# Lucaskabela/UNAST

Hardware: AMD Instinct MI355X
Metric: mel-frames/sec/node (train step, gen+disc) at B=32,T_mel=800; 1/2/4/8-GPU scaling (higher is better)
Workload: dtype bf16x3

## Files before the change

### unast_amd/csrc/panel.hip

```cpp
#include "common.h"
#include <algorithm>
#include "../../include/unast_hip.h"
#include <type_traits>

static unsigned long long* g_panel_stamps = nullptr;
#define PSUB 1024

struct PanelParams {
    const float* A; int lda;
    const unsigned char* W; size_t plane_bytes;
    float* C; int ldc;
    int M, N, K, ncg;
    const float* bias; const float* R; int ldr;
    const float* G; int ldg; float gate_scale;
    int act; uint32_t drop_thresh; float drop_scale; uint32_t seed, stream;
    int out_split;
    const float* gamma; const float* beta; float* Y; int ldy; float* mean; float* rstd; float eps;
    const float* Z; int ldz; float* part;
    unsigned long long* gate_bits;
    unsigned long long* stamps;
};

__device__ __forceinline__ void panel_wait_vm(int n) {
#define PW(k) asm volatile("s_waitcnt vmcnt(" #k ")" ::: "memory")
// ... 356 lines not shown
                        x += rr[r];
                        zv[rt][cg][c2][r] = x;
                        s1[rt] += x;
                    }
                }
            s1[rt] += __shfl_xor(s1[rt], 16, 64);
            s1[rt] += __shfl_xor(s1[rt], 32, 64);
        }
        if (g == 0) {
#pragma unroll
            for (int rt = 0; rt < RT; ++rt) sred[((rg * 2 + ch) * RT + rt) * 16 + l15] = s1[rt];
        }
        __syncthreads();
        float mu[RT], s2[RT];
#pragma unroll
        for (int rt = 0; rt < RT; ++rt) {
            mu[rt] = (s1[rt] + sred[((rg * 2 + (ch ^ 1)) * RT + rt) * 16 + l15]) * (1.f / 256.f);
            s2[rt] = 0.f;
#pragma unroll
            for (int cg = 0; cg < 4; ++cg)
#pragma unroll
                for (int c2 = 0; c2 < 2; ++c2)
#pragma unroll
                    for (int r = 0; r < 4; ++r) { const float d = zv[rt][cg][c2][r] - mu[rt]; s2[rt] += d * d; }
            s2[rt] += __shfl_xor(s2[rt], 16, 64);
            s2[rt] += __shfl_xor(s2[rt], 32, 64);
        }
        __syncthreads();
        if (g == 0) {
#pragma unroll
            for (int rt = 0; rt < RT; ++rt) sred[((rg * 2 + ch) * RT + rt) * 16 + l15] = s2[rt];
        }
        __syncthreads();
#pragma unroll
        for (int rt = 0; rt < RT; ++rt) {
            const int m = m_wave + 16 * rt + l15;
            const float rs = rsqrtf((s2[rt] + sred[((rg * 2 + (ch ^ 1)) * RT + rt) * 16 + l15]) * (1.f / 256.f) + p.eps);
            if (m >= p.M) continue;
            if (g == 0 && ch == 0) { p.mean[m] = mu[rt]; p.rstd[m] = rs; }
#pragma unroll
            for (int cg = 0; cg < 4; ++cg)
#pragma unroll
                for (int c2 = 0; c2 < 2; ++c2) {
                    const int n = 64 * cg + 32 * ch + 16 * c2 + 4 * g;
                    const float4 g4 = *reinterpret_cast<const float4*>(p.gamma + n), b4 = *reinterpret_cast<const float4*>(p.beta + n);
                    const float* z = zv[rt][cg][c2];
                    *reinterpret_cast<float4*>(p.C + (size_t)m * p.ldc + n) = make_float4(z[0], z[1], z[2], z[3]);
                    *reinterpret_cast<float4*>(p.Y + (size_t)m * p.ldy + n) =
                        make_float4((z[0] - mu[rt]) * rs * g4.x + b4.x, (z[1] - mu[rt]) * rs * g4.y + b4.y, (z[2] - mu[rt]) * rs * g4.z + b4.z, (z[3] - mu[rt]) * rs * g4.w + b4.w);
                }
        }
    } else {
        const bool late = ((wave >> 2) & 1) != 0;
        f32x4 acc[RT][2], pend[RT][2];
        zero(acc);
        for (int cg = 0; cg < p.ncg; ++cg) {
            group_sync(cg);
            if (!late && cg > 0) run_epilogue(cg - 1, pend);
            group_mma(cg, I0{}, IH{}, acc);
            if (late && cg > 0) run_epilogue(cg - 1, pend);
            group_mma(cg, IH{}, IK{}, acc);
            end_iteration();
#pragma unroll
            for (int rt = 0; rt < RT; ++rt) { pend[rt][0] = acc[rt][0]; pend[rt][1] = acc[rt][1]; }
            zero(acc);
        }
        run_epilogue(p.ncg - 1, pend);
    }
    asm volatile("s_waitcnt vmcnt(0)" ::: "memory");
#ifdef PANEL_STAMPS
    if (p.stamps && lane == 0) {
        stamp_sum[6] = panel_stamp() - t_begin;
        for (int k = 0; k < 8; ++k) p.stamps[((size_t)blockIdx.x * 8 + wave) * 8 + k] = stamp_sum[k];
    }
#endif
}

typedef __attribute__((ext_vector_type(16))) float f32x16_t;
__global__ __launch_bounds__(512, 1) void panel32_kernel(const PanelParams p) {
    constexpr int KSTEPS = 8, NW = 8, NT = 64 * NW, ROWS = 128;
    constexpr int NSUB = 8 * KSTEPS, GROUP = NSUB * PSUB, DMAX = NSUB / NW, RING = 2 * GROUP;
    static_assert(RING >= ROWS * 1024, "the A image borrows the ring");
    __shared__ __attribute__((aligned(16))) unsigned char smem[RING + 4096 + 1024];
    const int t = threadIdx.x, lane = t & 63, l31 = lane & 31, kh = lane >> 5;
    const int wave = __builtin_amdgcn_readfirstlane(t >> 6);
    __builtin_assume(wave >= 0 && wave < NW);
    const int rg = wave >> 1, ch = wave & 1;
    const int m_wg = blockIdx.x * ROWS, m_wave = m_wg + 32 * rg;
    const uint32_t rbase = p.drop_thresh ? rng_stream_base(p.seed, p.stream) : 0u;
    const __amdgpu_buffer_rsrc_t w_rsrc = __builtin_amdgcn_make_buffer_rsrc(const_cast<unsigned char*>(p.W), 0, 0x7FFFFFF0, 0x00020000);
    const int lane16 = lane * 16;
    auto issue_group = [&](int cg) {
#pragma unroll
        for (int q = 0; q < DMAX; ++q) {
            const int j = wave + NW * q;
            const int pl = j / (4 * KSTEPS), rem = j - pl * (4 * KSTEPS);
            const uint32_t soff = (uint32_t)pl * (uint32_t)p.plane_bytes + (uint32_t)(4 * cg * KSTEPS + rem) * PSUB;
            __builtin_amdgcn_raw_ptr_buffer_load_lds(w_rsrc, (__attribute__((address_space(3))) void*)(smem + (cg & 1) * GROUP + j * PSUB), 16, lane16, (int)soff, 0, 0);
        }
    };
    float* const sbias = reinterpret_cast<float*>(smem + RING);
    const uint32_t sbias_lds = (uint32_t)(uintptr_t)(__attribute__((address_space(3))) void*)sbias;
    const bool bias_lds = p.bias != nullptr;
    if (bias_lds) for (int i = t; i < 64 * p.ncg; i += NT) sbias[i] = (i < p.N) ? p.bias[i] : 0.f;

    bf16x8_t ah[16], al[16];
    {
        const __amdgpu_buffer_rsrc_t a_rsrc = __builtin_amdgcn_make_buffer_rsrc(const_cast<float*>(p.A), 0, 0x7FFFFFF0, 0x00020000);
#pragma unroll
        for (int q = 0; q < ROWS / NW; ++q) {
            const int r = wave * (ROWS / NW) + q;
            const int row = min(m_wg + r, p.M - 1);
            __builtin_amdgcn_raw_ptr_buffer_load_lds(a_rsrc, (__attribute__((address_space(3))) void*)(smem + r * 1024), 16, (lane ^ (r & 15)) << 4,
                                                     (int)((uint32_t)row * (uint32_t)p.lda * 4u), 0, 0);
        }
        asm volatile("s_waitcnt vmcnt(0)" ::: "memory");
        __syncthreads();
        const unsigned char* rowp = smem + (32 * rg + l31) * 1024;
        const int sw = l31 & 15;
#pragma unroll
        for (int ks = 0; ks < 16; ++ks) {
            const int c0 = 4 * ks + 2 * kh;
            const float4 a = *reinterpret_cast<const float4*>(rowp + ((c0 ^ sw) << 4));
            const float4 c = *reinterpret_cast<const float4*>(rowp + (((c0 + 1) ^ sw) << 4));
            u32x2 h0, l0, h1, l1;
            split4<3>(a, h0, l0);
            split4<3>(c, h1, l1);
            ah[ks] = __builtin_bit_cast(bf16x8_t, (u32x4){h0[0], h0[1], h1[0], h1[1]});
            al[ks] = __builtin_bit_cast(bf16x8_t, (u32x4){l0[0], l0[1], l1[0], l1[1]});
        }
        __syncthreads();
    }
    issue_group(0);

    const __amdgpu_buffer_rsrc_t c_rsrc = __builtin_amdgcn_make_buffer_rsrc(p.C, 0, (int)min((size_t)0x7FFFFFF0, ((size_t)(p.M - 1) * p.ldc + p.N) * 4), 0x00020000);
    const int m = m_wave + l31;
    const uint32_t c_voff = ((uint32_t)m * (uint32_t)p.ldc + (uint32_t)(32 * ch + 4 * kh)) * 4u;
    const uint32_t c_rkey = pcg_hash((uint32_t)m + rbase);
    auto epilogue = [&](int cg, const f32x16_t& ac, auto act_t, auto drop_t, auto split_t) {
        constexpr bool ACT = decltype(act_t)::value, DROP = decltype(drop_t)::value, SPLIT = decltype(split_t)::value;
        f32x4 b4[4];
#pragma unroll
        for (int j = 0; j < 4; ++j) b4[j] = (f32x4){0.f, 0.f, 0.f, 0.f};
        if (bias_lds) {
            const uint32_t ba = sbias_lds + 4u * (uint32_t)(64 * cg + 32 * ch + 4 * kh);
            asm volatile("ds_read_b128 %0, %4\n\tds_read_b128 %1, %4 offset:32\n\tds_read_b128 %2, %4 offset:64\n\tds_read_b128 %3, %4 offset:96\n\ts_waitcnt lgkmcnt(0)"
                         : "=&v"(b4[0]), "=&v"(b4[1]), "=&v"(b4[2]), "=&v"(b4[3]) : "v"(ba) : "memory");
        }
        const int soff = cg * 256;
#pragma unroll
        for (int j = 0; j < 4; ++j) {
            float v[4] = {ac[4 * j] + b4[j][0], ac[4 * j + 1] + b4[j][1], ac[4 * j + 2] + b4[j][2], ac[4 * j + 3] + b4[j][3]};
            if (ACT) {
#pragma unroll
                for (int r = 0; r < 4; ++r) asm("v_max_f32 %0, 0, %1" : "=v"(v[r]) : "v"(v[r]));
            }
            if (DROP) {
                const uint32_t n = (uint32_t)(64 * cg + 32 * ch + 8 * j + 4 * kh);
                const uint32_t h01 = rng_pair(c_rkey, n), h23 = rng_pair(c_rkey, n + 2u);
                v[0] = rng_keep_lo(h01, p.drop_thresh) ? v[0] * p.drop_scale : 0.f;
                v[1] = rng_keep_hi(h01, p.drop_thresh) ? v[1] * p.drop_scale : 0.f;
                v[2] = rng_keep_lo(h23, p.drop_thresh) ? v[2] * p.drop_scale : 0.f;
                v[3] = rng_keep_hi(h23, p.drop_thresh) ? v[3] * p.drop_scale : 0.f;
            }
            u32x4 o;
            if (SPLIT) {
                const uint4 sc = split_chunk(make_float4(v[0], v[1], v[2], v[3]));
                o = (u32x4){sc.x, sc.y, sc.z, sc.w};
            } else {
                o = (u32x4){__float_as_uint(v[0]), __float_as_uint(v[1]), __float_as_uint(v[2]), __float_as_uint(v[3])};
            }
            __builtin_amdgcn_raw_buffer_store_b128(o, c_rsrc, (int)(c_voff + (uint32_t)soff) + 32 * j, 0, 0);
        }
    };
    const int epi_kind = p.drop_thresh ? 1 : p.out_split ? 2 : p.act == 1 ? 3 : 4;
    int st_prev = 0, st_now = 0;
    auto run_epilogue = [&](int cg, const f32x16_t& ac) {
        using T = std::true_type; using F = std::false_type;
        __builtin_amdgcn_s_setprio(1);
        if (epi_kind == 1) epilogue(cg, ac, T{}, T{}, F{});
        else if (epi_kind == 2) epilogue(cg, ac, F{}, F{}, T{});
        else if (epi_kind == 3) epilogue(cg, ac, T{}, F{}, F{});
        else epilogue(cg, ac, F{}, F{}, F{});
        __builtin_amdgcn_s_setprio(0);
        st_now += 4;
    };
    auto group_sync = [&](int cg) {
        panel_wait_vm(st_prev);
        __builtin_amdgcn_s_barrier();
        if (cg + 1 < p.ncg) issue_group(cg + 1);
    };
    const int lane_off = (2 * ch + (l31 >> 4)) * KSTEPS * PSUB + (kh * 16 + (l31 & 15)) * 16;
    auto group_mma = [&](int cg, auto k0_t, auto k1_t, f32x16_t& ac) {
        constexpr int K0 = decltype(k0_t)::value, K1 = decltype(k1_t)::value;
        const unsigned char* base = smem + (cg & 1) * GROUP + lane_off;
        bf16x8_t bf[2][2];
        auto load_b = [&](int buf, int ks) {
            bf[buf][0] = *reinterpret_cast<const bf16x8_t*>(base + (ks >> 1) * PSUB + (ks & 1) * 512);
            bf[buf][1] = *reinterpret_cast<const bf16x8_t*>(base + 4 * KSTEPS * PSUB + (ks >> 1) * PSUB + (ks & 1) * 512);
        };
        load_b(K0 & 1, K0);
#pragma unroll
        for (int ks = K0; ks < K1; ++ks) {
            if (ks + 1 < K1) load_b((ks + 1) & 1, ks + 1);
            const bf16x8_t bh = bf[ks & 1][0], bl = bf[ks & 1][1];
            ac = __builtin_amdgcn_mfma_f32_32x32x16_bf16(bl, ah[ks], ac, 0, 0, 0);
            ac = __builtin_amdgcn_mfma_f32_32x32x16_bf16(bh, al[ks], ac, 0, 0, 0);
            ac = __builtin_amdgcn_mfma_f32_32x32x16_bf16(bh, ah[ks], ac, 0, 0, 0);
        }
    };
    using I0 = std::integral_constant<int, 0>; using IH = std::integral_constant<int, 8>; using IK = std::integral_constant<int, 16>;
    const bool late = ((wave >> 2) & 1) != 0;
    f32x16_t acc, pend;
#pragma unroll
    for (int i = 0; i < 16; ++i) { acc[i] = 0.f; pend[i] = 0.f; }
    for (int cg = 0; cg < p.ncg; ++cg) {
        group_sync(cg);
        if (!late && cg > 0) run_epilogue(cg - 1, pend);
        group_mma(cg, I0{}, IH{}, acc);
        if (late && cg > 0) run_epilogue(cg - 1, pend);
        group_mma(cg, IH{}, IK{}, acc);
        st_prev = st_now; st_now = 0;
        pend = acc;
#pragma unroll
        for (int i = 0; i < 16; ++i) acc[i] = 0.f;
    }
    run_epilogue(p.ncg - 1, pend);
    asm volatile("s_waitcnt vmcnt(0)" ::: "memory");
}

struct RetileDesc { int src_off, ld, transposed, N, K, n0, k0, ksteps; long long dst_off, plane_bytes; };

__global__ __launch_bounds__(256) void retile_kernel(const float* __restrict__ src_base, unsigned char* __restrict__ dst_base, const RetileDesc* __restrict__ descs) {
    __shared__ float tile[64][65];
    const RetileDesc d = descs[blockIdx.x];
    const float* src = src_base + d.src_off;
    const int t = threadIdx.x;
#pragma unroll
    for (int i = 0; i < 4; ++i) {
        const int idx = t + 256 * i, r = idx >> 4, c4 = (idx & 15) * 4;
        float v[4] = {0.f, 0.f, 0.f, 0.f};
        if (!d.transposed) {
            const int n = d.n0 + r;
            for (int e = 0; e < 4; ++e) if (n < d.N && d.k0 + c4 + e < d.K) v[e] = src[(size_t)n * d.ld + d.k0 + c4 + e];
            for (int e = 0; e < 4; ++e) tile[r][c4 + e] = v[e];
        } else {
            const int k = d.k0 + r;
            for (int e = 0; e < 4; ++e) if (k < d.K && d.n0 + c4 + e < d.N) v[e] = src[(size_t)k * d.ld + d.n0 + c4 + e];
            for (int e = 0; e < 4; ++e) tile[c4 + e][r] = v[e];
        }
    }
    __syncthreads();
#pragma unroll
    for (int i = 0; i < 2; ++i) {
        const int u = t + 256 * i;
        const int st = u >> 6, w = u & 63;
        const int ct = st >> 1, ksl = st & 1, gg = w >> 4, l = w & 15;
        const int ks = d.k0 / 32 + ksl;
        if (ks >= d.ksteps) continue;
        const int n = 16 * ct + l, k = 32 * ksl + 8 * gg;
        const float4 a = make_float4(tile[n][k], tile[n][k + 1], tile[n][k + 2], tile[n][k + 3]);
        const float4 c = make_float4(tile[n][k + 4], tile[n][k + 5], tile[n][k + 6], tile[n][k + 7]);
        u32x2 h0, l0, h1, l1;
        split4<3>(a, h0, l0);
        split4<3>(c, h1, l1);
        unsigned char* dst = dst_base + d.dst_off + ((size_t)((d.n0 / 16 + ct) * d.ksteps + ks)) * PSUB + w * 16;
        *reinterpret_cast<uint4*>(dst) = make_uint4(h0[0], h0[1], h1[0], h1[1]);
        *reinterpret_cast<uint4*>(dst + d.plane_bytes) = make_uint4(l0[0], l0[1], l1[0], l1[1]);
    }
}

extern "C" int unast_retile_weights(const float* src_base, void* dst_base, const void* descs_dev, int ndesc, hipStream_t stream) {
    UNAST_REQUIRE(src_base && dst_base && descs_dev && ndesc > 0, "unast_retile_weights: bad arguments");
    UNAST_REQUIRE((((uintptr_t)dst_base) & 15) == 0, "unast_retile_weights: destination must be 16-byte aligned");
    hipLaunchKernelGGL(retile_kernel, dim3(ndesc), dim3(256), 0, stream, src_base, (unsigned char*)dst_base, (const RetileDesc*)descs_dev);
    return unast_check_launch("unast_retile_weights");
}

template <int LN>
__global__ __launch_bounds__(1024, 4) void kpanel_kernel(const PanelParams p) {
    constexpr int NW = 16, ROWS = 128, WSLOT = 32768, ASLOT = 16384;
    __shared__ __attribute__((aligned(16))) unsigned char smem[3 * WSLOT + 3 * ASLOT + 1024 + 2048];
    const int t = threadIdx.x, lane = t & 63, l15 = lane & 15, g = lane >> 4;
    const int wave = __builtin_amdgcn_readfirstlane(t >> 6);
    __builtin_assume(wave >= 0 && wave < NW);
    const int rg = wave >> 2, ch = wave & 3;
    const int m_wg = blockIdx.x * ROWS, n_wg = blockIdx.y * 256;
    const int m_wave = m_wg + 32 * rg;
    const int KG = p.K >> 5;
#ifdef PANEL_STAMPS
    unsigned long long stamp_sum[8] = {0, 0, 0, 0, 0, 0, 0, 0};
    const unsigned long long t_begin = panel_stamp();
#endif
    const uint32_t rbase = p.drop_thresh ? rng_stream_base(p.seed, p.stream) : 0u;
    unsigned char* const aring = smem + 3 * WSLOT;

    const __amdgpu_buffer_rsrc_t w_rsrc = __builtin_amdgcn_make_buffer_rsrc(const_cast<unsigned char*>(p.W), 0, 0x7FFFFFF0, 0x00020000);
    const __amdgpu_buffer_rsrc_t a_rsrc = __builtin_amdgcn_make_buffer_rsrc(const_cast<float*>(p.A), 0, 0x7FFFFFF0, 0x00020000);
    const int lane16 = lane * 16;
    const int ar = 8 * wave + (lane >> 3);
    const uint32_t a_voff = ((uint32_t)min(m_wg + ar, p.M - 1) * (uint32_t)p.lda + 4u * (uint32_t)((lane & 7) ^ ((ar & 7) ^ ((ar >> 3) & 1)))) * 4u;
    const uint32_t w_soff0 = (uint32_t)((n_wg >> 4) + wave) * (uint32_t)(KG * PSUB);
    auto issue_group = [&](int kg, int slot) {
#pragma unroll
        for (int q = 0; q < 2; ++q)
            __builtin_amdgcn_raw_ptr_buffer_load_lds(w_rsrc, (__attribute__((address_space(3))) void*)(smem + slot * WSLOT + (q * 16 + wave) * PSUB), 16, lane16,
                                                     (int)((uint32_t)q * (uint32_t)p.plane_bytes + w_soff0 + (uint32_t)kg * PSUB), 0, 0);
        __builtin_amdgcn_raw_ptr_buffer_load_lds(a_rsrc, (__attribute__((address_space(3))) void*)(aring + slot * ASLOT + wave * 1024), 16, (int)a_voff, kg * 128, 0, 0);
    };
    float* const sbias = reinterpret_cast<float*>(smem + 3 * WSLOT + 3 * ASLOT);
    float* const sred = sbias + 256;
    if (t < 256) sbias[t] = p.bias ? p.bias[n_wg + t] : 0.f;
    issue_group(0, 0);
    if (KG > 1) issue_group(1, 1);

    f32x4 acc[2][4];
#pragma unroll
    for (int rt = 0; rt < 2; ++rt)
#pragma unroll
        for (int ct = 0; ct < 4; ++ct) acc[rt][ct] = (f32x4){0.f, 0.f, 0.f, 0.f};
    uint32_t a_rd[2][2];
#pragma unroll
    for (int rt = 0; rt < 2; ++rt) {
        const int r = 32 * rg + 16 * rt + l15, key = (r & 7) ^ ((r >> 3) & 1);
#pragma unroll
        for (int h = 0; h < 2; ++h) a_rd[rt][h] = (uint32_t)(r * 128 + (((2 * g + h) ^ key) << 4));
    }
    const uint32_t aring_lds = (uint32_t)(uintptr_t)(__attribute__((address_space(3))) void*)aring;
    const uint32_t wring_lds = (uint32_t)(uintptr_t)(__attribute__((address_space(3))) void*)smem + (uint32_t)(lane16 + (4 * ch) * PSUB);
    f32x4 raw[2][2];
    bf16x8_t b0h[2], b0l[2], b1h[2], b1l[2];
    bf16x8_t ah[2], al[2];
#define KP_READ_A(slot_) do { const uint32_t ab = aring_lds + (uint32_t)(slot_) * ASLOT; \
        asm volatile("ds_read_b128 %0, %4\n\tds_read_b128 %1, %5\n\tds_read_b128 %2, %6\n\tds_read_b128 %3, %7" \
                     : "=&v"(raw[0][0]), "=&v"(raw[0][1]), "=&v"(raw[1][0]), "=&v"(raw[1][1]) \
                     : "v"(ab + a_rd[0][0]), "v"(ab + a_rd[0][1]), "v"(ab + a_rd[1][0]), "v"(ab + a_rd[1][1]) : "memory"); } while (0)
#define KP_READ_W0(slot_) do { const uint32_t wb = wring_lds + (uint32_t)(slot_) * WSLOT; \
        asm volatile("ds_read_b128 %0, %4\n\tds_read_b128 %1, %4 offset:16384\n\tds_read_b128 %2, %4 offset:1024\n\tds_read_b128 %3, %4 offset:17408" \
                     : "=&v"(b0h[0]), "=&v"(b0l[0]), "=&v"(b0h[1]), "=&v"(b0l[1]) : "v"(wb) : "memory"); } while (0)
#define KP_READ_W1(slot_) do { const uint32_t wb = wring_lds + (uint32_t)(slot_) * WSLOT; \
        asm volatile("ds_read_b128 %0, %4 offset:2048\n\tds_read_b128 %1, %4 offset:18432\n\tds_read_b128 %2, %4 offset:3072\n\tds_read_b128 %3, %4 offset:19456" \
                     : "=&v"(b1h[0]), "=&v"(b1l[0]), "=&v"(b1h[1]), "=&v"(b1l[1]) : "v"(wb) : "memory"); } while (0)
    int slot = 0;
    if (KG > 1) asm volatile("s_waitcnt vmcnt(3)" ::: "memory"); else asm volatile("s_waitcnt vmcnt(0)" ::: "memory");
    __builtin_amdgcn_s_barrier();
    KP_READ_A(0);
    KP_READ_W0(0);
    if (KG > 2) issue_group(2, 2);
    for (int kg = 0; kg < KG; ++kg) {
        STAMP(ta);
        asm volatile("s_waitcnt lgkmcnt(4)" : "+v"(raw[0][0]), "+v"(raw[0][1]), "+v"(raw[1][0]), "+v"(raw[1][1]) :: "memory");
        STAMP(tb);
#pragma unroll
        for (int rt = 0; rt < 2; ++rt) {
            u32x2 h0, l0, h1, l1;
            split4<3>(make_float4(raw[rt][0][0], raw[rt][0][1], raw[rt][0][2], raw[rt][0][3]), h0, l0);
            split4<3>(make_float4(raw[rt][1][0], raw[rt][1][1], raw[rt][1][2], raw[rt][1][3]), h1, l1);
            ah[rt] = __builtin_bit_cast(bf16x8_t, (u32x4){h0[0], h0[1], h1[0], h1[1]});
            al[rt] = __builtin_bit_cast(bf16x8_t, (u32x4){l0[0], l0[1], l1[0], l1[1]});
        }
        KP_READ_W1(slot);
        asm volatile("s_waitcnt lgkmcnt(4)" : "+v"(b0h[0]), "+v"(b0l[0]), "+v"(b0h[1]), "+v"(b0l[1]) :: "memory");
        STAMP(tc);
#pragma unroll
        for (int ct = 0; ct < 2; ++ct)
#pragma unroll
            for (int rt = 0; rt < 2; ++rt) {
                acc[rt][ct] = mfma16(b0l[ct], ah[rt], acc[rt][ct]);
                acc[rt][ct] = mfma16(b0h[ct], al[rt], acc[rt][ct]);
                acc[rt][ct] = mfma16(b0h[ct], ah[rt], acc[rt][ct]);
            }
        asm volatile("" :: "v"(acc[0][0]), "v"(acc[1][0]), "v"(acc[0][1]), "v"(acc[1][1]));
        asm volatile("s_waitcnt lgkmcnt(0)" : "+v"(b1h[0]), "+v"(b1l[0]), "+v"(b1h[1]), "+v"(b1l[1]) :: "memory");
        STAMP(td);
        if (kg + 1 < KG) {
            if (kg + 2 < KG) asm volatile("s_waitcnt vmcnt(3)" ::: "memory"); else asm volatile("s_waitcnt vmcnt(0)" ::: "memory");
            STAMP(te);
            __builtin_amdgcn_s_barrier();
            STAMP(tf);
            const int nslot = slot == 2 ? 0 : slot + 1;
            KP_READ_A(nslot);
            KP_READ_W0(nslot);
            if (kg + 3 < KG) issue_group(kg + 3, slot);
            STAMP(tg);
            STAMP_ADD(2, td, te); STAMP_ADD(3, te, tf); STAMP_ADD(4, tf, tg);
            slot = nslot;
        }
#pragma unroll
        for (int ct = 0; ct < 2; ++ct)
#pragma unroll
            for (int rt = 0; rt < 2; ++rt) {
                acc[rt][2 + ct] = mfma16(b1l[ct], ah[rt], acc[rt][2 + ct]);
                acc[rt][2 + ct] = mfma16(b1h[ct], al[rt], acc[rt][2 + ct]);
                acc[rt][2 + ct] = mfma16(b1h[ct], ah[rt], acc[rt][2 + ct]);
            }
#ifdef PANEL_STAMPS
        asm volatile("" :: "v"(acc[0][0]), "v"(acc[1][3]));
#endif
        STAMP(th);
        STAMP_ADD(0, ta, tb); STAMP_ADD(1, tb, tc); STAMP_ADD(5, tc, td);
    }
#undef KP_READ_A
#undef KP_READ_W0
#undef KP_READ_W1
#ifdef PANEL_STAMPS
    const unsigned long long t_loop = panel_stamp();
#endif
    __syncthreads();
    if constexpr (LN == 2) {
        float* const red = reinterpret_cast<float*>(smem);
        float xh[2][4][4], mu[2], rs[2], s1[2], s2[2];
#pragma unroll
        for (int rt = 0; rt < 2; ++rt) {
            const int mr = m_wave + 16 * rt + l15, m = min(mr, p.M - 1);
            mu[rt] = p.mean[m]; rs[rt] = p.rstd[m];
            s1[rt] = 0.f; s2[rt] = 0.f;
#pragma unroll
            for (int ct = 0; ct < 4; ++ct) {
                const int n = 64 * ch + 16 * ct + 4 * g;
                const float4 r4 = p.R ? *reinterpret_cast<const float4*>(p.R + (size_t)m * p.ldr + n) : make_float4(0.f, 0.f, 0.f, 0.f);
                const float4 z4 = *reinterpret_cast<const float4*>(p.Z + (size_t)m * p.ldz + n);
                const float4 g4 = *reinterpret_cast<const float4*>(p.gamma + n);
                const float rr[4] = {r4.x, r4.y, r4.z, r4.w}, zz[4] = {z4.x, z4.y, z4.z, z4.w}, gm[4] = {g4.x, g4.y, g4.z, g4.w};
#pragma unroll
                for (int r = 0; r < 4; ++r) {
                    const float dy = mr < p.M ? acc[rt][ct][r] + rr[r] : 0.f;
                    const float x = (zz[r] - mu[rt]) * rs[rt];
                    const float gg = dy * gm[r];
                    acc[rt][ct][r] = dy; xh[rt][ct][r] = x;
                    s1[rt] += gg; s2[rt] += gg * x;
                }
            }
            s1[rt] += __shfl_xor(s1[rt], 16, 64); s1[rt] += __shfl_xor(s1[rt], 32, 64);
            s2[rt] += __shfl_xor(s2[rt], 16, 64); s2[rt] += __shfl_xor(s2[rt], 32, 64);
        }
        if (g == 0) {
#pragma unroll
            for (int rt = 0; rt < 2; ++rt) {
                red[ch * 128 + 32 * rg + 16 * rt + l15] = s1[rt];
                red[512 + ch * 128 + 32 * rg + 16 * rt + l15] = s2[rt];
            }
        }
        __syncthreads();
        float cg[4][4], cb[4][4];
#pragma unroll
        for (int ct = 0; ct < 4; ++ct)
#pragma unroll
            for (int r = 0; r < 4; ++r) { cg[ct][r] = 0.f; cb[ct][r] = 0.f; }
#pragma unroll
        for (int rt = 0; rt < 2; ++rt) {
            const int r0 = 32 * rg + 16 * rt + l15, m = m_wg + r0;
            const float c1 = ((red[r0] + red[128 + r0]) + (red[256 + r0] + red[384 + r0])) * (1.f / 256.f);
            const float c2 = ((red[512 + r0] + red[640 + r0]) + (red[768 + r0] + red[896 + r0])) * (1.f / 256.f);
            uint32_t rkey = 0;
            if (p.drop_thresh) rkey = pcg_hash((uint32_t)min(m, p.M - 1) + rbase);
#pragma unroll
            for (int ct = 0; ct < 4; ++ct) {
                const int n = 64 * ch + 16 * ct + 4 * g;
                const float4 g4 = *reinterpret_cast<const float4*>(p.gamma + n);
                const float gm[4] = {g4.x, g4.y, g4.z, g4.w};
                float o[4], od[4];
#pragma unroll
                for (int r = 0; r < 4; ++r) {
                    o[r] = rs[rt] * (acc[rt][ct][r] * gm[r] - c1 - xh[rt][ct][r] * c2);
                    od[r] = (!p.drop_thresh || rng_keep(rkey, (uint32_t)(n + r), p.drop_thresh)) ? o[r] * p.drop_scale : 0.f;
                    cg[ct][r] += acc[rt][ct][r] * xh[rt][ct][r];
                    cb[ct][r] += acc[rt][ct][r];
                }
                if (m < p.M) {
                    *reinterpret_cast<float4*>(p.C + (size_t)m * p.ldc + n) = make_float4(o[0], o[1], o[2], o[3]);
                    if (p.Y) *reinterpret_cast<float4*>(p.Y + (size_t)m * p.ldy + n) = make_float4(od[0], od[1], od[2], od[3]);
                }
            }
        }
        __syncthreads();
#pragma unroll
        for (int ct = 0; ct < 4; ++ct)
#pragma unroll
            for (int r = 0; r < 4; ++r) {
                float a = cg[ct][r], b = cb[ct][r];
#pragma unroll
                for (int o = 1; o < 16; o <<= 1) { a += __shfl_xor(a, o, 64); b += __shfl_xor(b, o, 64); }
                if (l15 == 0) {
                    const int n = 64 * ch + 16 * ct + 4 * g + r;
                    red[rg * 256 + n] = a;
                    red[1024 + rg * 256 + n] = b;
                }
            }
        __syncthreads();
        if (p.part && t < 512) {
            const int q = t >> 8, n = t & 255;
            const float* rp = red + q * 1024 + n;
            p.part[((size_t)blockIdx.x * 2 + q) * 256 + n] = (rp[0] + rp[256]) + (rp[512] + rp[768]);
        }
    } else if constexpr (!LN) {
#pragma unroll
        for (int rt = 0; rt < 2; ++rt) {
            const int m = m_wave + 16 * rt + l15;
            if (m >= p.M) continue;
#pragma unroll
            for (int ct = 0; ct < 4; ++ct) {
                const int nl = 64 * ch + 16 * ct + 4 * g, n = n_wg + nl;
                const float4 b4 = *reinterpret_cast<const float4*>(sbias + nl);
                float4 o = make_float4(acc[rt][ct][0] + b4.x, acc[rt][ct][1] + b4.y, acc[rt][ct][2] + b4.z, acc[rt][ct][3] + b4.w);
                if (p.R) { const float4 r4 = *reinterpret_cast<const float4*>(p.R + (size_t)m * p.ldr + n); o.x += r4.x; o.y += r4.y; o.z += r4.z; o.w += r4.w; }
                *reinterpret_cast<float4*>(p.C + (size_t)m * p.ldc + n) = o;
            }
        }
    } else {
        float mu[2], s1[2], s2[2];
#pragma unroll
        for (int rt = 0; rt < 2; ++rt) {
            const int m = min(m_wave + 16 * rt + l15, p.M - 1);
            uint32_t rkey = 0;
            if (p.drop_thresh) rkey = pcg_hash((uint32_t)m + rbase);
            s1[rt] = 0.f;
#pragma unroll
            for (int ct = 0; ct < 4; ++ct) {
                const int n = 64 * ch + 16 * ct + 4 * g;
                const float4 b4 = *reinterpret_cast<const float4*>(sbias + n);
                const float4 r4 = p.R ? *reinterpret_cast<const float4*>(p.R + (size_t)m * p.ldr + n) : make_float4(0.f, 0.f, 0.f, 0.f);
                const float bb[4] = {b4.x, b4.y, b4.z, b4.w}, rr[4] = {r4.x, r4.y, r4.z, r4.w};
#pragma unroll
                for (int r = 0; r < 4; ++r) {
                    float x = acc[rt][ct][r] + bb[r];
                    if (p.drop_thresh) x = rng_keep(rkey, (uint32_t)(n + r), p.drop_thresh) ? x * p.drop_scale : 0.f;
                    x += rr[r];
                    acc[rt][ct][r] = x;
                    s1[rt] += x;
                }
            }
            s1[rt] += __shfl_xor(s1[rt], 16, 64);
            s1[rt] += __shfl_xor(s1[rt], 32, 64);
        }
        if (g == 0) {
#pragma unroll
            for (int rt = 0; rt < 2; ++rt) sred[ch * 128 + 32 * rg + 16 * rt + l15] = s1[rt];
        }
        __syncthreads();
#pragma unroll
        for (int rt = 0; rt < 2; ++rt) {
            const int r0 = 32 * rg + 16 * rt + l15;
            mu[rt] = ((sred[r0] + sred[128 + r0]) + (sred[256 + r0] + sred[384 + r0])) * (1.f / 256.f);
            s2[rt] = 0.f;
#pragma unroll
            for (int ct = 0; ct < 4; ++ct)
#pragma unroll
                for (int r = 0; r < 4; ++r) { const float d = acc[rt][ct][r] - mu[rt]; s2[rt] += d * d; }
            s2[rt] += __shfl_xor(s2[rt], 16, 64);
            s2[rt] += __shfl_xor(s2[rt], 32, 64);
        }
        __syncthreads();
        if (g == 0) {
#pragma unroll
            for (int rt = 0; rt < 2; ++rt) sred[ch * 128 + 32 * rg + 16 * rt + l15] = s2[rt];
        }
        __syncthreads();
#pragma unroll
        for (int rt = 0; rt < 2; ++rt) {
            const int r0 = 32 * rg + 16 * rt + l15, m = m_wg + r0;
            const float rs = rsqrtf(((sred[r0] + sred[128 + r0]) + (sred[256 + r0] + sred[384 + r0])) * (1.f / 256.f) + p.eps);
            if (m >= p.M) continue;
            if (g == 0 && ch == 0) { p.mean[m] = mu[rt]; p.rstd[m] = rs; }
#pragma unroll
            for (int ct = 0; ct < 4; ++ct) {
                const int n = 64 * ch + 16 * ct + 4 * g;
                const float4 g4 = *reinterpret_cast<const float4*>(p.gamma + n), b4 = *reinterpret_cast<const float4*>(p.beta + n);
                const f32x4 z = acc[rt][ct];
                *reinterpret_cast<float4*>(p.C + (size_t)m * p.ldc + n) = make_float4(z[0], z[1], z[2], z[3]);
                *reinterpret_cast<float4*>(p.Y + (size_t)m * p.ldy + n) =
                    make_float4((z[0] - mu[rt]) * rs * g4.x + b4.x, (z[1] - mu[rt]) * rs * g4.y + b4.y, (z[2] - mu[rt]) * rs * g4.z + b4.z, (z[3] - mu[rt]) * rs * g4.w + b4.w);
            }
        }
    }
#ifdef PANEL_STAMPS
    if (p.stamps && lane == 0) {
        const unsigned long long t_end = panel_stamp();
        stamp_sum[6] = t_end - t_begin; stamp_sum[7] = t_end - t_loop;
        for (int k = 0; k < 8; ++k) p.stamps[((size_t)(blockIdx.x * gridDim.y + blockIdx.y) * 16 + wave) * 8 + k] = stamp_sum[k];
    }
#endif
}

template <int KSTEPS>
static void panel_launch(const PanelParams& p, int rows, int ln, hipStream_t s) {
    const int r = rows == 1128 ? 128 : rows;
    dim3 grid((p.M + r - 1) / r);
    if (rows == 1128) {
        if (ln) hipLaunchKernelGGL((panel_kernel<KSTEPS, 1, 1, 16>), grid, dim3(1024), 0, s, p);
        else    hipLaunchKernelGGL((panel_kernel<KSTEPS, 1, 0, 16>), grid, dim3(1024), 0, s, p);
    } else if (ln) {
        if (rows == 128) hipLaunchKernelGGL((panel_kernel<KSTEPS, 2, 1, 8>), grid, dim3(512), 0, s, p);
        else             hipLaunchKernelGGL((panel_kernel<KSTEPS, 1, 1, 8>), grid, dim3(512), 0, s, p);
    } else {
        if (rows == 128) hipLaunchKernelGGL((panel_kernel<KSTEPS, 2, 0, 8>), grid, dim3(512), 0, s, p);
        else             hipLaunchKernelGGL((panel_kernel<KSTEPS, 1, 0, 8>), grid, dim3(512), 0, s, p);
    }
}

extern "C" int64_t unast_panel_gemm_lnbwd_ws_floats(int M) { return (int64_t)((M + 127) / 128) * 2 * 256; }

extern "C" int unast_panel_gemm_lnbwd(const float* A, int lda, const void* w_planes, int64_t plane_bytes, int M, int K, const float* R, int ldr,
                                      const float* z, int ldz, const float* mean, const float* rstd, const float* gamma,
                                      float* dz, int lddz, float* dz_drop, int lddrop, float* part, int64_t part_floats,
                                      float drop_p, unsigned int seed, unsigned int stream_id, hipStream_t stream) {
    UNAST_REQUIRE(A && w_planes && z && mean && rstd && gamma && dz && M > 0, "unast_panel_gemm_lnbwd: null pointer");
    UNAST_REQUIRE(K > 256 && (K & 63) == 0 && (lda & 3) == 0 && (lddz & 3) == 0 && (ldz & 3) == 0 && (!R || (ldr & 3) == 0) && (!dz_drop || (lddrop & 3) == 0) &&
                  ((((uintptr_t)A) | ((uintptr_t)dz) | ((uintptr_t)w_planes) | ((uintptr_t)z) | ((uintptr_t)R) | ((uintptr_t)dz_drop) | ((uintptr_t)gamma)) & 15) == 0,
                  "unast_panel_gemm_lnbwd: needs K > 256, K %% 64 == 0, 16-byte row strides and aligned operands (K=%d)", K);
    UNAST_REQUIRE(!part || part_floats >= unast_panel_gemm_lnbwd_ws_floats(M), "unast_panel_gemm_lnbwd: partials buffer too small");
    UNAST_REQUIRE(dz_drop || drop_p <= 0.f, "unast_panel_gemm_lnbwd: dropout needs the second output");
    {
        const size_t ld_max = (size_t)std::max(std::max(lda, lddz), std::max(std::max(R ? ldr : 0, ldz), dz_drop ? lddrop : 0));
        UNAST_REQUIRE(((size_t)M + 127) / 128 * 128 * ld_max * 4 < (size_t)0x7FFFFFF0u, "unast_panel_gemm_lnbwd: operand exceeds the 2 GiB a buffer descriptor addresses");
    }
    PanelParams q = {};
    q.stamps = nullptr;
    q.A = A; q.lda = lda; q.W = (const unsigned char*)w_planes; q.plane_bytes = (size_t)plane_bytes; q.C = dz; q.ldc = lddz; q.M = M; q.N = 256; q.K = K; q.ncg = 4;
    q.R = R; q.ldr = ldr; q.Z = z; q.ldz = ldz; q.mean = const_cast<float*>(mean); q.rstd = const_cast<float*>(rstd); q.gamma = gamma;
    q.Y = dz_drop; q.ldy = lddrop; q.part = part;
    q.drop_thresh = dz_drop ? drop_threshold(drop_p) : 0u; q.drop_scale = drop_p > 0.f ? 1.f / (1.f - drop_p) : 1.f; q.seed = seed; q.stream = stream_id;
    hipLaunchKernelGGL((kpanel_kernel<2>), dim3((M + 127) / 128, 1), dim3(1024), 0, stream, q);
    return unast_check_launch("unast_panel_gemm_lnbwd");
}

extern "C" int unast_panel_debug_stamps(void* dev_buf) { g_panel_stamps = (unsigned long long*)dev_buf; return 0; }

extern "C" int unast_panel_gemm(const float* A, int lda, const void* w_planes, int64_t plane_bytes, float* C, int ldc, int M, int N, int K,
                                const float* bias, const float* R, int ldr, const float* G, int ldg, float gate_scale, int act,
                                float drop_p, unsigned int seed, unsigned int stream_id, int out_split,
                                const float* ln_gamma, const float* ln_beta, float* Y, int ldy, float* mean, float* rstd, float eps,
                                void* gate_bits, int rows_per_wg, hipStream_t stream) {
    UNAST_REQUIRE(A && w_planes && C && M > 0 && N > 0 && K >= 4, "unast_panel_gemm: bad arguments");
    {
        const size_t ld_max = (size_t)std::max(std::max(lda, ldc), std::max(R ? ldr : 0, Y ? ldy : 0));
        UNAST_REQUIRE(((size_t)M + 127) / 128 * 128 * ld_max * 4 < (size_t)0x7FFFFFF0u, "unast_panel_gemm: operand of %d rows x %zu floats exceeds the 2 GiB a buffer descriptor addresses (use unast_gemm)", M, ld_max);
    }
    if (K > 256) {
        UNAST_REQUIRE((K & 63) == 0 && (N & 255) == 0 && (lda & 3) == 0 && (ldc & 3) == 0 && ((((uintptr_t)A) | ((uintptr_t)C) | ((uintptr_t)w_planes)) & 15) == 0,
                      "unast_panel_gemm: K > 256 needs K %% 64 == 0, N %% 256 == 0, 16-byte row strides and aligned operands (N=%d K=%d)", N, K);
        UNAST_REQUIRE(!G && !act && !out_split && !gate_bits, "unast_panel_gemm: K > 256 serves the plain, residual and LayerNorm epilogues only");
        UNAST_REQUIRE(!R || ((ldr & 3) == 0 && (((uintptr_t)R) & 15) == 0), "unast_panel_gemm: residual operand must be 16-byte addressable");
        const int lnk = ln_gamma != nullptr;
        UNAST_REQUIRE(lnk || drop_p <= 0.f, "unast_panel_gemm: K > 256: dropout only inside the LayerNorm epilogue");
        UNAST_REQUIRE(!lnk || (N == 256 && ln_beta && Y && mean && rstd && (ldy & 3) == 0), "unast_panel_gemm: the LayerNorm epilogue needs N = 256, Y / mean / rstd and 16-byte row strides");
        PanelParams q = {};
        q.stamps = g_panel_stamps;
        q.A = A; q.lda = lda; q.W = (const unsigned char*)w_planes; q.plane_bytes = (size_t)plane_bytes; q.C = C; q.ldc = ldc; q.M = M; q.N = N; q.K = K; q.ncg = N / 64;
        q.bias = bias; q.R = R; q.ldr = ldr; q.drop_thresh = drop_threshold(drop_p); q.drop_scale = drop_p > 0.f ? 1.f / (1.f - drop_p) : 1.f; q.seed = seed; q.stream = stream_id;
        q.gamma = ln_gamma; q.beta = ln_beta; q.Y = Y; q.ldy = ldy; q.mean = mean; q.rstd = rstd; q.eps = eps;
        dim3 grid((M + 127) / 128, N / 256);
        if (lnk) hipLaunchKernelGGL((kpanel_kernel<1>), grid, dim3(1024), 0, stream, q);
        else     hipLaunchKernelGGL((kpanel_kernel<0>), grid, dim3(1024), 0, stream, q);
        return unast_check_launch("unast_panel_gemm");
    }
    UNAST_REQUIRE((K & 3) == 0 && K <= 256 && (lda & 3) == 0 && ((((uintptr_t)A) | ((uintptr_t)C) | ((uintptr_t)w_planes)) & 15) == 0,
                  "unast_panel_gemm: needs K %% 4 == 0, K <= 256, lda %% 4 == 0 and 16-byte aligned operands (K=%d lda=%d)", K, lda);
    UNAST_REQUIRE(rows_per_wg == 0 || rows_per_wg == 64 || rows_per_wg == 128 || rows_per_wg == 1128 || rows_per_wg == 2128, "unast_panel_gemm: rows_per_wg is 64, 128, 1128 (128 rows, 16 waves), 2128 (128 rows, 32x32x16 tiles) or 0 (auto)");
    UNAST_REQUIRE(!out_split || ((N & 3) == 0 && (ldc & 3) == 0), "unast_panel_gemm: out_split needs N %% 4 == 0 and ldc %% 4 == 0");
    const int ln = ln_gamma != nullptr;
    UNAST_REQUIRE(!ln || (N == 256 && ln_beta && Y && mean && rstd && (ldc & 3) == 0 && (ldy & 3) == 0 && !G && !act && !out_split &&
                          (!R || (ldr & 3) == 0)), "unast_panel_gemm: the LayerNorm epilogue needs N = 256, Y / mean / rstd and 16-byte row strides");
    PanelParams p;
    p.A = A; p.lda = lda; p.W = (const unsigned char*)w_planes; p.plane_bytes = (size_t)plane_bytes; p.C = C; p.ldc = ldc;
    p.M = M; p.N = N; p.K = K; p.ncg = (N + 63) / 64;
    p.bias = bias; p.R = R; p.ldr = ldr; p.G = G; p.ldg = ldg; p.gate_scale = gate_scale; p.act = act;
    p.drop_thresh = drop_threshold(drop_p); p.drop_scale = drop_p > 0.f ? 1.f / (1.f - drop_p) : 1.f; p.seed = seed; p.stream = stream_id;
    p.out_split = out_split;
    p.gate_bits = (unsigned long long*)gate_bits;
    UNAST_REQUIRE(!gate_bits || ((N & 63) == 0 && !G && !R && !ln && (ldc & 3) == 0 && (((uintptr_t)gate_bits) & 15) == 0 && (act == 1 ? (!out_split && N <= 1024) : (!bias && !out_split && drop_p <= 0.f))),
                  "unast_panel_gemm: gate_bits needs N %% 64 == 0 and either the relu (+ dropout) epilogue (writes them) or the plain gated one (reads them)");
    p.stamps = g_panel_stamps;
    p.gamma = ln_gamma; p.beta = ln_beta; p.Y = Y; p.ldy = ldy; p.mean = mean; p.rstd = rstd; p.eps = eps;
    UNAST_REQUIRE((ldc & 3) == 0 || !out_split, "unast_panel_gemm: ldc");
    if (rows_per_wg == 2128) {
        UNAST_REQUIRE(K == 256 && (N & 63) == 0 && (ldc & 3) == 0 && !R && !G && !ln && !gate_bits && N <= 1024 && !(out_split && (act || drop_p > 0.f)) && !(drop_p > 0.f && act != 1),
                      "unast_panel_gemm: rows_per_wg = 2128 serves K = 256, N %% 64 == 0 and the plain / relu / relu + dropout / split epilogues only");
        hipLaunchKernelGGL(panel32_kernel, dim3((M + 127) / 128), dim3(512), 0, stream, p);
        return unast_check_launch("unast_panel_gemm");
    }
    const int ksteps = (K + 31) / 32;
    UNAST_REQUIRE(ksteps != 8 || K == 256, "unast_panel_gemm: 224 < K < 256 is not built (the 8-k-step form copies whole 1-KB activation rows by LDS-DMA; K=%d)", K);
    const int rt = rows_per_wg ? rows_per_wg : (M >= 16384 ? 128 : 64);
    switch (ksteps) {
        case 8: panel_launch<8>(p, rt, ln, stream); break;
        case 4: panel_launch<4>(p, rt, ln, stream); break;
        case 3: panel_launch<3>(p, rt, ln, stream); break;
        case 2: panel_launch<2>(p, rt, ln, stream); break;
        case 1: panel_launch<1>(p, rt, ln, stream); break;
        case 6: panel_launch<6>(p, rt, ln, stream); break;
        default: return unast_set_error(UNAST_ERR_ARG, "unast_panel_gemm: K = %d (ceil(K/32) = %d k-steps) is not built (1, 2, 3, 4, 6, 8)", K, ksteps);
    }
    return unast_check_launch("unast_panel_gemm");
}

UNAST_DEFINE_RNG_EPOCH_SETTER(panel)
```

Measured before the change: 936,300.

## Split A tile into bf16 hi/lo once in LDS instead of per-wave

Each wave now converts its own freshly loaded fp32 A chunk into bf16 hi/lo halves and writes them back into the LDS ring before the barrier. The main loop can then use the A fragments directly as bf16 operands. This removes the split arithmetic that the four column-waves each repeated on the same A rows. The A load is issued first in each group so a partial vmcnt wait covers only A, and the k-loop is unrolled by two with ping-pong fragment registers. The cost is extra LDS reads, writes and lgkmcnt waits on the critical path before each barrier. The unroll also assumes an even number of K groups.

```diff
diff --git a/unast_amd/csrc/panel.hip b/unast_amd/csrc/panel.hip
--- a/unast_amd/csrc/panel.hip
+++ b/unast_amd/csrc/panel.hip
@@ -682,11 +682,11 @@
     const uint32_t a_voff = ((uint32_t)min(m_wg + ar, p.M - 1) * (uint32_t)p.lda + 4u * (uint32_t)((lane & 7) ^ ((ar & 7) ^ ((ar >> 3) & 1)))) * 4u;
     const uint32_t w_soff0 = (uint32_t)((n_wg >> 4) + wave) * (uint32_t)(KG * PSUB);
     auto issue_group = [&](int kg, int slot) {
+        __builtin_amdgcn_raw_ptr_buffer_load_lds(a_rsrc, (__attribute__((address_space(3))) void*)(aring + slot * ASLOT + wave * 1024), 16, (int)a_voff, kg * 128, 0, 0);
 #pragma unroll
         for (int q = 0; q < 2; ++q)
             __builtin_amdgcn_raw_ptr_buffer_load_lds(w_rsrc, (__attribute__((address_space(3))) void*)(smem + slot * WSLOT + (q * 16 + wave) * PSUB), 16, lane16,
                                                      (int)((uint32_t)q * (uint32_t)p.plane_bytes + w_soff0 + (uint32_t)kg * PSUB), 0, 0);
-        __builtin_amdgcn_raw_ptr_buffer_load_lds(a_rsrc, (__attribute__((address_space(3))) void*)(aring + slot * ASLOT + wave * 1024), 16, (int)a_voff, kg * 128, 0, 0);
     };
     float* const sbias = reinterpret_cast<float*>(smem + 3 * WSLOT + 3 * ASLOT);
     float* const sred = sbias + 256;
@@ -708,12 +708,22 @@
     }
     const uint32_t aring_lds = (uint32_t)(uintptr_t)(__attribute__((address_space(3))) void*)aring;
     const uint32_t wring_lds = (uint32_t)(uintptr_t)(__attribute__((address_space(3))) void*)smem + (uint32_t)(lane16 + (4 * ch) * PSUB);
-    f32x4 raw[2][2];
+    f32x4 fr0[2][2], fr1[2][2];
     bf16x8_t b0h[2], b0l[2], b1h[2], b1l[2];
     bf16x8_t ah[2], al[2];
-#define KP_READ_A(slot_) do { const uint32_t ab = aring_lds + (uint32_t)(slot_) * ASLOT; \
+    f32x4 cv;
+    const int a_key = (ar & 7) ^ ((ar >> 3) & 1), a_c = (lane & 7) ^ a_key;
+    const uint32_t cv_rd = aring_lds + (uint32_t)(wave * 1024 + lane16);
+    const uint32_t cv_pair = aring_lds + (uint32_t)(wave * 1024 + ((lane & ~1) << 4) + 8 * (a_c & 1));
+    const uint32_t cv_hi = cv_pair + 16u * (uint32_t)(a_key & 1), cv_lo = cv_pair + 16u * (uint32_t)((a_key & 1) ^ 1);
+#define KP_SPLIT_READ(slot_) asm volatile("ds_read_b128 %0, %1" : "=&v"(cv) : "v"(cv_rd + (uint32_t)(slot_) * ASLOT) : "memory")
+#define KP_SPLIT_WRITE(slot_) do { const uint4 sc = split_chunk(make_float4(cv[0], cv[1], cv[2], cv[3])); \
+        const u32x2 shi = {sc.x, sc.y}, slo = {sc.z, sc.w}; \
+        asm volatile("ds_write_b64 %0, %2\n\tds_write_b64 %1, %3" \
+                     :: "v"(cv_hi + (uint32_t)(slot_) * ASLOT), "v"(cv_lo + (uint32_t)(slot_) * ASLOT), "v"(shi), "v"(slo) : "memory"); } while (0)
+#define KP_READ_A(dst_, slot_) do { const uint32_t ab = aring_lds + (uint32_t)(slot_) * ASLOT; \
         asm volatile("ds_read_b128 %0, %4\n\tds_read_b128 %1, %5\n\tds_read_b128 %2, %6\n\tds_read_b128 %3, %7" \
-                     : "=&v"(raw[0][0]), "=&v"(raw[0][1]), "=&v"(raw[1][0]), "=&v"(raw[1][1]) \
+                     : "=&v"(dst_[0][0]), "=&v"(dst_[0][1]), "=&v"(dst_[1][0]), "=&v"(dst_[1][1]) \
                      : "v"(ab + a_rd[0][0]), "v"(ab + a_rd[0][1]), "v"(ab + a_rd[1][0]), "v"(ab + a_rd[1][1]) : "memory"); } while (0)
 #define KP_READ_W0(slot_) do { const uint32_t wb = wring_lds + (uint32_t)(slot_) * WSLOT; \
         asm volatile("ds_read_b128 %0, %4\n\tds_read_b128 %1, %4 offset:16384\n\tds_read_b128 %2, %4 offset:1024\n\tds_read_b128 %3, %4 offset:17408" \
@@ -722,25 +732,33 @@
         asm volatile("ds_read_b128 %0, %4 offset:2048\n\tds_read_b128 %1, %4 offset:18432\n\tds_read_b128 %2, %4 offset:3072\n\tds_read_b128 %3, %4 offset:19456" \
                      : "=&v"(b1h[0]), "=&v"(b1l[0]), "=&v"(b1h[1]), "=&v"(b1l[1]) : "v"(wb) : "memory"); } while (0)
     int slot = 0;
+    if (KG > 1) asm volatile("s_waitcnt vmcnt(5)" ::: "memory"); else asm volatile("s_waitcnt vmcnt(2)" ::: "memory");
+    KP_SPLIT_READ(0);
+    asm volatile("s_waitcnt lgkmcnt(0)" : "+v"(cv) :: "memory");
+    KP_SPLIT_WRITE(0);
     if (KG > 1) asm volatile("s_waitcnt vmcnt(3)" ::: "memory"); else asm volatile("s_waitcnt vmcnt(0)" ::: "memory");
+    asm volatile("s_waitcnt lgkmcnt(0)" ::: "memory");
     __builtin_amdgcn_s_barrier();
-    KP_READ_A(0);
+    KP_READ_A(fr0, 0);
     KP_READ_W0(0);
     if (KG > 2) issue_group(2, 2);
-    for (int kg = 0; kg < KG; ++kg) {
+    auto group = [&](const int kg, f32x4 (&raw)[2][2], f32x4 (&rawn)[2][2]) __attribute__((always_inline)) {
         STAMP(ta);
         asm volatile("s_waitcnt lgkmcnt(4)" : "+v"(raw[0][0]), "+v"(raw[0][1]), "+v"(raw[1][0]), "+v"(raw[1][1]) :: "memory");
         STAMP(tb);
 #pragma unroll
         for (int rt = 0; rt < 2; ++rt) {
-            u32x2 h0, l0, h1, l1;
-            split4<3>(make_float4(raw[rt][0][0], raw[rt][0][1], raw[rt][0][2], raw[rt][0][3]), h0, l0);
-            split4<3>(make_float4(raw[rt][1][0], raw[rt][1][1], raw[rt][1][2], raw[rt][1][3]), h1, l1);
-            ah[rt] = __builtin_bit_cast(bf16x8_t, (u32x4){h0[0], h0[1], h1[0], h1[1]});
-            al[rt] = __builtin_bit_cast(bf16x8_t, (u32x4){l0[0], l0[1], l1[0], l1[1]});
-        }
+            ah[rt] = __builtin_bit_cast(bf16x8_t, raw[rt][0]);
+            al[rt] = __builtin_bit_cast(bf16x8_t, raw[rt][1]);
+        }
+        const int nslot = slot == 2 ? 0 : slot + 1;
+        const bool more = kg + 1 < KG;
+        if (more) {
+            if (kg + 2 < KG) asm volatile("s_waitcnt vmcnt(5)" ::: "memory"); else asm volatile("s_waitcnt vmcnt(2)" ::: "memory");
+        }
+        KP_SPLIT_READ(nslot);
         KP_READ_W1(slot);
-        asm volatile("s_waitcnt lgkmcnt(4)" : "+v"(b0h[0]), "+v"(b0l[0]), "+v"(b0h[1]), "+v"(b0l[1]) :: "memory");
+        asm volatile("s_waitcnt lgkmcnt(5)" : "+v"(b0h[0]), "+v"(b0l[0]), "+v"(b0h[1]), "+v"(b0l[1]) :: "memory");
         STAMP(tc);
 #pragma unroll
         for (int ct = 0; ct < 2; ++ct)
@@ -751,15 +769,16 @@
                 acc[rt][ct] = mfma16(b0h[ct], ah[rt], acc[rt][ct]);
             }
         asm volatile("" :: "v"(acc[0][0]), "v"(acc[1][0]), "v"(acc[0][1]), "v"(acc[1][1]));
-        asm volatile("s_waitcnt lgkmcnt(0)" : "+v"(b1h[0]), "+v"(b1l[0]), "+v"(b1h[1]), "+v"(b1l[1]) :: "memory");
+        asm volatile("s_waitcnt lgkmcnt(0)" : "+v"(b1h[0]), "+v"(b1l[0]), "+v"(b1h[1]), "+v"(b1l[1]), "+v"(cv) :: "memory");
         STAMP(td);
-        if (kg + 1 < KG) {
+        if (more) {
+            KP_SPLIT_WRITE(nslot);
             if (kg + 2 < KG) asm volatile("s_waitcnt vmcnt(3)" ::: "memory"); else asm volatile("s_waitcnt vmcnt(0)" ::: "memory");
+            asm volatile("s_waitcnt lgkmcnt(0)" ::: "memory");
             STAMP(te);
             __builtin_amdgcn_s_barrier();
             STAMP(tf);
-            const int nslot = slot == 2 ? 0 : slot + 1;
-            KP_READ_A(nslot);
+            KP_READ_A(rawn, nslot);
             KP_READ_W0(nslot);
             if (kg + 3 < KG) issue_group(kg + 3, slot);
             STAMP(tg);
@@ -779,7 +798,13 @@
 #endif
         STAMP(th);
         STAMP_ADD(0, ta, tb); STAMP_ADD(1, tb, tc); STAMP_ADD(5, tc, td);
-    }
+    };
+    for (int kg = 0; kg < KG; kg += 2) {
+        group(kg, fr0, fr1);
+        group(kg + 1, fr1, fr0);
+    }
+#undef KP_SPLIT_READ
+#undef KP_SPLIT_WRITE
 #undef KP_READ_A
 #undef KP_READ_W0
 #undef KP_READ_W1
```

Result: no change. 944,100, median of 6 (+0.8%).
